# linxihui/NNLM

Measured on AMD Instinct MI355X. Metric: nnmf iterations/sec + final MSE, dense A 20000x10000 k=50, 1/2/4/8 GPU, higher is better.
Workload: dtype f32 (A fp32; cross-product operands 22-bit split-fp16 pairs; Gram / sweeps fp64); 1 GPU; nnmf(A, k=50) MSE+SCD on 20000x10000 dense A (BASELINE.json configs[1]); n=20000, m=10000, k=50, method=1, inner_max_iter=50, trace=2, protocol=default, rel_tol=-1, parallelism=1 GPU

## Files before the change

include/nnlm_mi355x.h:

```cpp
#ifndef NNLM_MI355X_H
#define NNLM_MI355X_H

#include <stddef.h>

#ifdef __cplusplus
extern "C" {
#endif

#define NNLM_ABI_VERSION 1

#define NNLM_OK 0
#define NNLM_ERR_ARG 1
#define NNLM_ERR_HIP 2
#define NNLM_ERR_INTERRUPT 3
#define NNLM_ERR_COMM 4
#define NNLM_ERR_UNSUPPORTED 5

#define NNLM_PREC_F32 0
#define NNLM_PREC_F64 1

typedef struct nnlm_callbacks {
    void *ctx;
    int (*check_interrupt)(void *ctx);
    void (*progress)(void *ctx, unsigned done, unsigned total);
// ... 169 lines not shown
int nnlm_c_nnmf_holdout_batch(const double *A, int n, int m, const long long *colptr, const int *rowidx, unsigned B, const unsigned *k,
                              const double *W_init, const double *H_init, const double alpha[3], const double beta[3], unsigned max_iter,
                              double rel_tol, int n_threads, int verbose, int show_warning, unsigned inner_max_iter, double inner_rel_tol,
                              int method, unsigned trace, double *W_out, double *H_out, double *mse_error, double *mkl_error,
                              double *target_error, double *average_epoch, int *n_trace, unsigned *n_iteration, int *warned,
                              double *holdout_mse, double *holdout_mkl, const nnlm_callbacks *cb);

int nnlm_svd(nnlm_handle *h, unsigned l, unsigned power_iters, const double *omega);
int nnlm_debug_set_svd_rotate(int form);
int nnlm_get_svd(nnlm_handle *h, unsigned k, double *sigma, double *U, double *Vt);
int nnlm_set_factors_nndsvd(nnlm_handle *h, unsigned k, int variant);
int nnlm_set_factors_nndsvd_batch(nnlm_handle *h, unsigned B, const unsigned *k, int variant);

int nnlm_profile_enable(nnlm_handle *h, int on);
int nnlm_profile_get(nnlm_handle *h, const char *name, double *total_ms, long long *launches);
int nnlm_profile_reset(nnlm_handle *h);

#define NNLM_COMM_ID_BYTES 128
#define NNLM_FORM_COLS 0
#define NNLM_FORM_REDUCE 1
int nnlm_comm_unique_id(char id[NNLM_COMM_ID_BYTES]);
int nnlm_comm_init(nnlm_handle *h, const char id[NNLM_COMM_ID_BYTES], int rank, int nranks);
int nnlm_comm_set_form(nnlm_handle *h, int form);
int nnlm_comm_info(nnlm_handle *h, int *rank, int *nranks);
int nnlm_shard_range(int n, int m, int precision, int which, int rank, int nranks, int *begin, int *end);
int nnlm_shard_cols(int ncols, int rank, int nranks, int *cpr, int *col0, int *col1);
int nnlm_debug_partial(nnlm_handle *h, int which, double *G_out, double *C_out);

int nnlm_debug_phase(nnlm_handle *h, int which, int phase, const double reg[3], unsigned inner_max_iter,
                     double inner_rel_tol, int method);
int nnlm_debug_exchange(nnlm_handle **handles, int nranks, int which, int stage);
int nnlm_debug_set_cus(int cus);
int nnlm_debug_set_xprod_waves(int waves);
int nnlm_debug_set_a_stream(int nt_from_stage);
int nnlm_xprod_plan(int ldc, int stages, int k, int cus, int force_waves, int out[8]);
int nnlm_kl_plan(int p, int k, int precision, int mask_words, int out[8]);
int nnlm_debug_alloc_limit(size_t bytes);
int nnlm_debug_poison_workspaces(int on);
int nnlm_get_info(nnlm_handle *h, const char *key, double *value);

#ifdef __cplusplus
}
#endif
#endif
```

nnlm_amd/_lib.py:

```python
from __future__ import annotations

import ctypes as C
import os

import numpy as np

_HERE = os.path.dirname(os.path.abspath(__file__))
LIB_PATH = os.path.join(_HERE, "libnnlm_mi355x.so")

NNLM_OK = 0
ERR_ARG = 1
ERR_UNSUPPORTED = 5
BATCH_MAX = 64
PREC_F32 = 0
PREC_F64 = 1
COMM_ID_BYTES = 128
FORM_COLS = 0
FORM_REDUCE = 1
FORMS = {"cols": FORM_COLS, "reduce": FORM_REDUCE}

EXPORTS = [
    "nnlm_trace_capacity", "nnlm_c_nnmf", "nnlm_c_nnlm", "nnlm_create", "nnlm_destroy", "nnlm_last_error",
    "nnlm_abi_version", "nnlm_set_matrix", "nnlm_matrix_info", "nnlm_set_factors", "nnlm_get_factors",
    "nnlm_half_step", "nnlm_iterate", "nnlm_run", "nnlm_take_sweeps", "nnlm_errors", "nnlm_sync", "nnlm_profile_enable",
    "nnlm_profile_get", "nnlm_profile_reset", "nnlm_comm_unique_id", "nnlm_comm_init", "nnlm_comm_info",
    "nnlm_shard_range", "nnlm_shard_cols", "nnlm_debug_partial", "nnlm_debug_phase", "nnlm_debug_exchange",
    "nnlm_comm_set_form", "nnlm_debug_set_cus", "nnlm_debug_set_xprod_waves", "nnlm_debug_set_a_stream", "nnlm_xprod_plan", "nnlm_kl_plan", "nnlm_get_info", "nnlm_debug_alloc_limit", "nnlm_debug_poison_workspaces", "nnlm_release_caches",
    "nnlm_set_matrix_csc", "nnlm_c_nnmf_csc", "nnlm_c_nnlm_csc",
    "nnlm_set_matrix_csc_missing", "nnlm_c_nnmf_csc_missing", "nnlm_c_nnlm_csc_missing",
    "nnlm_set_matrix_csc_kl", "nnlm_c_nnmf_csc_kl", "nnlm_c_nnlm_csc_kl",
    "nnlm_set_factors_batch", "nnlm_get_factors_batch", "nnlm_run_batch", "nnlm_c_nnmf_batch",
    "nnlm_set_matrix_holdout", "nnlm_holdout_errors", "nnlm_c_nnmf_holdout_batch",
    "nnlm_set_matrix_device", "nnlm_set_factors_device", "nnlm_get_factors_device",
    "nnlm_predict_entries", "nnlm_top_n",
    "nnlm_set_matrix_csc_batch", "nnlm_c_nnmf_csc_batch",
    "nnlm_set_matrix_csc_kl_batch", "nnlm_c_nnmf_csc_kl_batch",
    "nnlm_set_matrix_csc_missing_batch", "nnlm_c_nnmf_csc_missing_batch",
    "nnlm_set_matrix_sparse_device", "nnlm_debug_sparse_resident",
    "nnlm_set_matrix_csc_weighted", "nnlm_c_nnmf_csc_weighted", "nnlm_c_nnlm_csc_weighted",
    "nnlm_set_matrix_sparse_device_weighted", "nnlm_debug_sparse_resident_weighted",
    "nnlm_svd", "nnlm_get_svd", "nnlm_set_factors_nndsvd", "nnlm_set_factors_nndsvd_batch", "nnlm_debug_set_svd_rotate",
]
NNDSVD_VARIANTS = {"nndsvd": 0, "nndsvda": 1}
TOPN_MAX = 128
BY = {"column": 0, "row": 1}


class NnlmError(RuntimeError):
    def __init__(self, code, msg):
        super().__init__(f"libnnlm_mi355x error {code}: {msg}")
        self.code = code


class DevMatrix(C.Structure):
    _fields_ = [("ptr", C.c_void_p), ("dtype", C.c_int), ("row_stride", C.c_longlong), ("col_stride", C.c_longlong)]


class DevSparse(C.Structure):
    _fields_ = [("ptr", C.c_void_p), ("idx", C.c_void_p), ("val", C.c_void_p), ("ptr_dtype", C.c_int), ("idx_dtype", C.c_int),
                ("val_dtype", C.c_int), ("layout", C.c_int), ("nnz", C.c_longlong)]
# ... 88 lines not shown
    lib.nnlm_errors.argtypes = [vp, dp, dp, dp]
    lib.nnlm_sync.restype = C.c_int
    lib.nnlm_sync.argtypes = [vp]
    lib.nnlm_profile_enable.restype = C.c_int
    lib.nnlm_profile_enable.argtypes = [vp, C.c_int]
    lib.nnlm_profile_reset.restype = C.c_int
    lib.nnlm_profile_reset.argtypes = [vp]
    lib.nnlm_profile_get.restype = C.c_int
    lib.nnlm_profile_get.argtypes = [vp, C.c_char_p, dp, C.POINTER(C.c_longlong)]
    lib.nnlm_comm_unique_id.restype = C.c_int
    lib.nnlm_comm_unique_id.argtypes = [C.c_char_p]
    lib.nnlm_comm_init.restype = C.c_int
    lib.nnlm_comm_init.argtypes = [vp, C.c_char_p, C.c_int, C.c_int]
    lib.nnlm_comm_info.restype = C.c_int
    lib.nnlm_comm_info.argtypes = [vp, ip, ip]
    lib.nnlm_shard_range.restype = C.c_int
    lib.nnlm_shard_range.argtypes = [C.c_int, C.c_int, C.c_int, C.c_int, C.c_int, C.c_int, ip, ip]
    lib.nnlm_shard_cols.restype = C.c_int
    lib.nnlm_shard_cols.argtypes = [C.c_int, C.c_int, C.c_int, ip, ip, ip]
    lib.nnlm_debug_partial.restype = C.c_int
    lib.nnlm_debug_partial.argtypes = [vp, C.c_int, dp, dp]
    lib.nnlm_debug_phase.restype = C.c_int
    lib.nnlm_debug_phase.argtypes = [vp, C.c_int, C.c_int, dp, C.c_uint, C.c_double, C.c_int]
    lib.nnlm_debug_exchange.restype = C.c_int
    lib.nnlm_debug_exchange.argtypes = [C.POINTER(vp), C.c_int, C.c_int, C.c_int]
    lib.nnlm_comm_set_form.restype = C.c_int
    lib.nnlm_comm_set_form.argtypes = [vp, C.c_int]
    lib.nnlm_debug_set_cus.restype = C.c_int
    lib.nnlm_debug_set_cus.argtypes = [C.c_int]
    lib.nnlm_debug_set_xprod_waves.restype = C.c_int
    lib.nnlm_debug_set_xprod_waves.argtypes = [C.c_int]
    lib.nnlm_debug_set_a_stream.restype = C.c_int
    lib.nnlm_debug_set_a_stream.argtypes = [C.c_int]
    lib.nnlm_xprod_plan.restype = C.c_int
    lib.nnlm_xprod_plan.argtypes = [C.c_int, C.c_int, C.c_int, C.c_int, C.c_int, ip]
    lib.nnlm_kl_plan.restype = C.c_int
    lib.nnlm_kl_plan.argtypes = [C.c_int, C.c_int, C.c_int, C.c_int, ip]
    lib.nnlm_debug_alloc_limit.restype = C.c_int
    lib.nnlm_debug_alloc_limit.argtypes = [C.c_size_t]
    lib.nnlm_debug_poison_workspaces.restype = C.c_int
    lib.nnlm_debug_poison_workspaces.argtypes = [C.c_int]
    lib.nnlm_release_caches.restype = C.c_int
    lib.nnlm_release_caches.argtypes = []
    lib.nnlm_get_info.restype = C.c_int
    lib.nnlm_get_info.argtypes = [vp, C.c_char_p, dp]
    up = C.POINTER(C.c_uint)
    lib.nnlm_set_factors_batch.restype = C.c_int
    lib.nnlm_set_factors_batch.argtypes = [vp, C.c_uint, up, dp, dp]
    lib.nnlm_get_factors_batch.restype = C.c_int
    lib.nnlm_get_factors_batch.argtypes = [vp, dp, dp]
    lib.nnlm_run_batch.restype = C.c_int
    lib.nnlm_run_batch.argtypes = lib.nnlm_run.argtypes
    lib.nnlm_c_nnmf_batch.restype = C.c_int
    lib.nnlm_c_nnmf_batch.argtypes = [dp, C.c_int, C.c_int, C.c_uint, up, dp, dp, dp, dp, C.c_uint, C.c_double, C.c_int, C.c_int, C.c_int,
                                      C.c_uint, C.c_double, C.c_int, C.c_uint, dp, dp, dp, dp, dp, dp, ip, up, ip, C.POINTER(Callbacks)]
    lib.nnlm_c_nnmf_csc_batch.restype = C.c_int
    lib.nnlm_c_nnmf_csc_batch.argtypes = [C.c_int, C.c_int, lp, ip, dp] + lib.nnlm_c_nnmf_batch.argtypes[3:]
    lib.nnlm_set_matrix_csc_batch.restype = C.c_int
    lib.nnlm_set_matrix_csc_batch.argtypes = lib.nnlm_set_matrix_csc.argtypes
    lib.nnlm_c_nnmf_csc_kl_batch.restype = C.c_int
    lib.nnlm_c_nnmf_csc_kl_batch.argtypes = lib.nnlm_c_nnmf_csc_batch.argtypes
    lib.nnlm_set_matrix_csc_kl_batch.restype = C.c_int
    lib.nnlm_set_matrix_csc_kl_batch.argtypes = lib.nnlm_set_matrix_csc.argtypes
    lib.nnlm_set_matrix_csc_missing_batch.restype = C.c_int
    lib.nnlm_set_matrix_csc_missing_batch.argtypes = lib.nnlm_set_matrix_csc.argtypes + [lp, ip]
    lib.nnlm_c_nnmf_csc_missing_batch.restype = C.c_int
# ... 893 lines not shown
        cols = self.m if which == 1 else self.n
        G = np.zeros((self.k, self.k), order="F")
        Cm = np.zeros((self.k, cols), order="F")
        self._ck(self._lib.nnlm_debug_partial(self._h, int(which), _dp(G), _dp(Cm)))
        return np.ascontiguousarray(G), np.ascontiguousarray(Cm)

    def comm_info(self):
        r, n = C.c_int(0), C.c_int(0)
        self._ck(self._lib.nnlm_comm_info(self._h, C.byref(r), C.byref(n)))
        return r.value, n.value


def shard_range(n, m, precision, which, rank, nranks):
    b, e = C.c_int(0), C.c_int(0)
    _check(load().nnlm_shard_range(int(n), int(m), int(precision), int(which), int(rank), int(nranks), C.byref(b), C.byref(e)))
    return b.value, e.value


def shard_cols(ncols, rank, nranks):
    cpr, c0, c1 = C.c_int(0), C.c_int(0), C.c_int(0)
    _check(load().nnlm_shard_cols(int(ncols), int(rank), int(nranks), C.byref(cpr), C.byref(c0), C.byref(c1)))
    return cpr.value, c0.value, c1.value


def debug_exchange(handles, which, stage):
    arr = (C.c_void_p * len(handles))(*[h._h for h in handles])
    _check(load().nnlm_debug_exchange(arr, len(handles), int(which), int(stage)))


def debug_set_cus(cus: int):
    _check(load().nnlm_debug_set_cus(int(cus)))


def debug_set_svd_rotate(form: int):
    _check(load().nnlm_debug_set_svd_rotate(int(form)))


def debug_set_xprod_waves(waves: int):
    _check(load().nnlm_debug_set_xprod_waves(int(waves)))


A_STREAM_NONE = 2**31 - 1


def debug_set_a_stream(nt_from_stage: int):
    _check(load().nnlm_debug_set_a_stream(int(nt_from_stage)))


def xprod_plan(ldc, stages, k, cus, force_waves=0):
    out = (C.c_int * 8)()
    _check(load().nnlm_xprod_plan(int(ldc), int(stages), int(k), int(cus), int(force_waves), out))
    return dict(zip(("waves", "splits", "stages_per_split", "tiles", "blocks", "pieces", "lds_bytes"), list(out)[:7]))


KL_TILE2, KL_TILE1, KL_REG64, KL_STREAM = 0, 1, 2, 3


def kl_plan(p, k, precision, mask_words=0):
    out = (C.c_int * 8)()
    _check(load().nnlm_kl_plan(int(p), int(k), int(precision), int(mask_words), out))
    return dict(zip(("kernel", "pieces_exact", "pieces", "cols", "lds_bytes", "last_waves"), list(out)[:6]))


def debug_alloc_limit(nbytes: int):
    _check(load().nnlm_debug_alloc_limit(int(nbytes)))

# ... 14 lines not shown
```

nnlm_amd/csrc/nnlm_mi355x.hip:

```cpp
#include "../../include/nnlm_mi355x.h"
#include "common.h"
#include "k_batch.h"
#include "k_errors.h"
#include "k_generic.h"
#include "k_gram.h"
#include "k_ingest.h"
#include "k_kl.h"
#include "k_missing.h"
#include "k_prep.h"
#include "k_sweep.h"
#include "k_sweep_q.h"
#include "k_xprod.h"
#include "k_xprod16.h"
#include "tu_sweepq.h"
#include "tu_svd.h"
#include "tu_topn.h"

#include <dlfcn.h>
#include <rccl/rccl.h>

#include <algorithm>
#include <atomic>
#include <chrono>
#include <climits>
// ... 119 lines not shown
    double *spg_buf = nullptr;
    size_t spg_buf_bytes = 0;
    int spg_chunks = 0;
    int spg_workers = 0;
    unsigned long long *sweeps = nullptr;
    int sw_active = 0;
    double *host_res = nullptr;

    int rank = 0, nranks = 1;
    void *comm = nullptr;
    bool sharded = false;
    double *pack_send = nullptr;
    double *pack_all = nullptr;
    size_t pack_elems = 0;
    double *sweepq_img = nullptr;
    bool x16 = false;
    uint32_t *A16 = nullptr, *A16T = nullptr, *Y16 = nullptr;
    unsigned *maxbits = nullptr;
    int sg_which = -1, sg_par = 0, sg_nslabs = 0;
    int sg_other = -1;
    int sg_prev = -1;
    bool sg_request = false;
    double *sg_slabs = nullptr;
    int mb_par = 0;
    bool pack_ready = false;
    int *scal_exp = nullptr;
    float *What = nullptr;
    double *What64 = nullptr;
    uint32_t *W16c = nullptr, *H16c = nullptr;
    bool fuse_err = false;
    int cus_device = 0;
    int xprod_waves = 0;
    int a_stream = -1;
    int a_stream_last = -1;
    int xp_err_splits = 0;
    int xp_waves[2] = {0, 0}, xp_splits[2] = {0, 0};
    int fused_nb = 0;
    bool err_hook = false, err_need_pen = true, err_launched = false;
    unsigned *err_zero_word = nullptr;
    unsigned long long *sweeps_tmp = nullptr;

    int bB = 0, row_pad = 0;
    std::vector<int> bk, boff;
    int *boff_dev = nullptr;
    double *bG = nullptr;
    unsigned long long *bsweeps = nullptr;
    double *bpart = nullptr;
    size_t bpart_elems = 0;
    double *bres = nullptr;
    double *bsp_Hrow = nullptr;
    double *bsp_part = nullptr;
    int bspg_pairs = 0;

    bool holdout = false;
    long long ho_nnz = 0;
    long long *ho_cptr = nullptr;
    int *ho_ridx = nullptr, *ho_cidx = nullptr;
    void *ho_val = nullptr;

    int topn_slices = 0;

    int svd_l = 0, svd_LP = 0, svd_kept = 0;
    double *svdU = nullptr, *svdVt = nullptr;
    std::vector<double> svd_sigma;
    double svd_mean = 0.0;
    bool svd_mean_known = false;
// ... 117 lines not shown
static Rccl g_rccl;

static int rccl_load()
{
    if (g_rccl.lib) return NNLM_OK;
    void *lib = dlopen("librccl.so.1", RTLD_NOW | RTLD_GLOBAL);
    if (!lib) lib = dlopen("librccl.so", RTLD_NOW | RTLD_GLOBAL);
    if (!lib) lib = dlopen("/opt/rocm/lib/librccl.so.1", RTLD_NOW | RTLD_GLOBAL);
    if (!lib) return fail(nullptr, NNLM_ERR_COMM, "cannot load librccl: %s", dlerror());
    g_rccl.GetUniqueId = (decltype(g_rccl.GetUniqueId))dlsym(lib, "ncclGetUniqueId");
    g_rccl.CommInitRank = (decltype(g_rccl.CommInitRank))dlsym(lib, "ncclCommInitRank");
    g_rccl.AllReduce = (decltype(g_rccl.AllReduce))dlsym(lib, "ncclAllReduce");
    g_rccl.AllGather = (decltype(g_rccl.AllGather))dlsym(lib, "ncclAllGather");
    g_rccl.CommDestroy = (decltype(g_rccl.CommDestroy))dlsym(lib, "ncclCommDestroy");
    g_rccl.GetErrorString = (decltype(g_rccl.GetErrorString))dlsym(lib, "ncclGetErrorString");
    if (!g_rccl.GetUniqueId || !g_rccl.CommInitRank || !g_rccl.AllReduce || !g_rccl.AllGather || !g_rccl.CommDestroy)
        return fail(nullptr, NNLM_ERR_COMM, "librccl lacks a required symbol");
    g_rccl.lib = lib;
    return NNLM_OK;
}

extern "C" int nnlm_abi_version(void) { return NNLM_ABI_VERSION; }

extern "C" const char *nnlm_last_error(const nnlm_handle *h) { return h ? h->err.c_str() : g_last_error.c_str(); }

extern "C" unsigned nnlm_trace_capacity(unsigned max_iter, unsigned trace)
{
    if (trace < 1) trace = 1;
    return (unsigned)std::ceil((double)max_iter / (double)trace) + 1;
}

static std::atomic<int> g_debug_cus{0};
static std::atomic<int> g_debug_a_stream{-1};
static std::atomic<int> g_debug_xprod_waves{0};
static std::mutex g_bounce_mu;
static double *g_bounce[2] = {nullptr, nullptr};
static size_t g_bounce_bytes = 0;
static bool g_bounce_busy = false, g_bounce_atexit = false;
static void bounce_release_at_exit()
{
    for (int b = 0; b < 2; b++)
        if (g_bounce[b]) (void)hipHostFree(g_bounce[b]);
    g_bounce[0] = g_bounce[1] = nullptr;
    g_bounce_bytes = 0;
}
static bool bounce_acquire(size_t bytes, double *out[2], bool *cached)
{
    {
        std::lock_guard<std::mutex> lk(g_bounce_mu);
        if (!g_bounce_busy) {
            if (g_bounce_bytes < bytes) {
                for (int b = 0; b < 2; b++)
                    if (g_bounce[b]) (void)hipHostFree(g_bounce[b]);
                g_bounce[0] = g_bounce[1] = nullptr;
                g_bounce_bytes = 0;
                if (hipHostMalloc(&g_bounce[0], bytes) != hipSuccess || hipHostMalloc(&g_bounce[1], bytes) != hipSuccess) {
                    (void)hipGetLastError();
                    for (int b = 0; b < 2; b++)
                        if (g_bounce[b]) (void)hipHostFree(g_bounce[b]);
                    g_bounce[0] = g_bounce[1] = nullptr;
                    return false;
                }
                g_bounce_bytes = bytes;
                if (!g_bounce_atexit) {
                    g_bounce_atexit = true;
                    atexit(bounce_release_at_exit);
// ... 46 lines not shown
{
    g_debug_alloc_limit = bytes;
    return NNLM_OK;
}

static std::atomic<int> g_debug_poison{0};

extern "C" int nnlm_debug_poison_workspaces(int on)
{
    g_debug_poison = on ? 1 : 0;
    return NNLM_OK;
}

static hipError_t poison_new_gram(void *p, size_t bytes, hipStream_t st)
{
    if (!g_debug_poison.load(std::memory_order_relaxed)) return hipSuccess;
    return hipMemsetAsync(p, 0xFF, bytes, st);
}

extern "C" int nnlm_debug_set_xprod_waves(int waves)
{
    if (waves != 0 && waves != 8 && waves != 10) return fail(nullptr, NNLM_ERR_ARG, "nnlm_debug_set_xprod_waves: %d (0, 8 or 10)", waves);
    g_debug_xprod_waves = waves;
    return NNLM_OK;
}

extern "C" int nnlm_debug_set_a_stream(int nt_from_stage)
{
    if (nt_from_stage < -1) return fail(nullptr, NNLM_ERR_ARG, "nnlm_debug_set_a_stream: %d (-1, or a stage >= 0)", nt_from_stage);
    g_debug_a_stream = nt_from_stage;
    return NNLM_OK;
}

extern "C" int nnlm_debug_set_cus(int cus)
{
    if (cus < 0) return fail(nullptr, NNLM_ERR_ARG, "nnlm_debug_set_cus: %d", cus);
    g_debug_cus = cus;
    return NNLM_OK;
}

struct HandleRes {
    bool valid = false;
    int device = -1, cus = 0;
    hipStream_t stream = nullptr, stream_e = nullptr;
    hipEvent_t ev_hdone = nullptr, ev_err = nullptr, ev_xdone = nullptr;
    double *scal = nullptr, *host_res = nullptr, *sweepq_img = nullptr;
    unsigned long long *sweeps = nullptr, *sweeps_tmp = nullptr;
    unsigned *maxbits = nullptr;
    int *scal_exp = nullptr;
};
static std::mutex g_res_mu;
static HandleRes g_res;
static bool g_res_atexit = false;
static void handle_res_destroy(HandleRes &r)
{
    (void)hipFree(r.scal), (void)hipFree(r.sweeps), (void)hipHostFree(r.host_res), (void)hipFree(r.sweeps_tmp), (void)hipFree(r.sweepq_img);
    (void)hipFree(r.maxbits), (void)hipFree(r.scal_exp);
    if (r.ev_hdone) (void)hipEventDestroy(r.ev_hdone);
    if (r.ev_err) (void)hipEventDestroy(r.ev_err);
    if (r.ev_xdone) (void)hipEventDestroy(r.ev_xdone);
    if (r.stream_e) (void)hipStreamDestroy(r.stream_e);
    if (r.stream) (void)hipStreamDestroy(r.stream);
    r = HandleRes{};
}
static void handle_res_release_at_exit()
{
    if (g_res.valid) handle_res_destroy(g_res);
}

extern "C" int nnlm_create(nnlm_handle **out, int device, int precision)
{
    if (!out) return fail(nullptr, NNLM_ERR_ARG, "nnlm_create: out is NULL");
    *out = nullptr;
    if (precision != NNLM_PREC_F32 && precision != NNLM_PREC_F64) return fail(nullptr, NNLM_ERR_ARG, "nnlm_create: unknown precision %d", precision);
    int ndev = 0;
    hipError_t e = hipGetDeviceCount(&ndev);
    if (e != hipSuccess || ndev <= 0)
        return fail(nullptr, NNLM_ERR_HIP, "nnlm_create: no HIP device available (%s); libnnlm_mi355x has no CPU path", e != hipSuccess ? hipGetErrorString(e) : "device count 0");
    if (device < 0 || device >= ndev) return fail(nullptr, NNLM_ERR_ARG, "nnlm_create: device %d out of range (0..%d)", device, ndev - 1);
    HIPCHK(nullptr, hipSetDevice(device));
    HandleRes res;
    {
        std::lock_guard<std::mutex> lk(g_res_mu);
        if (g_res.valid && g_res.device == device) {
            res = g_res;
            g_res = HandleRes{};
        }
    }
    if (res.valid) {
        nnlm_handle *h = new nnlm_handle();
        h->device = device;
        h->prec = precision;
        h->cus = h->cus_device = res.cus;
        if (const int dc = g_debug_cus.load(std::memory_order_relaxed); dc > 0) h->cus = dc;
        h->xprod_waves = g_debug_xprod_waves.load(std::memory_order_relaxed);
        h->a_stream = g_debug_a_stream.load(std::memory_order_relaxed);
        h->stream = res.stream, h->stream_e = res.stream_e;
        h->ev_hdone = res.ev_hdone, h->ev_err = res.ev_err, h->ev_xdone = res.ev_xdone;
        h->scal = res.scal, h->sweeps = res.sweeps, h->host_res = res.host_res, h->sweeps_tmp = res.sweeps_tmp, h->sweepq_img = res.sweepq_img;
        h->maxbits = res.maxbits, h->scal_exp = res.scal_exp;
        const bool alive = hipMemsetAsync(h->sweeps, 0, 2 * sizeof(unsigned long long), h->stream) == hipSuccess &&
                           hipMemsetAsync(h->scal_exp, 0, 4 * sizeof(int), h->stream) == hipSuccess &&
                           hipMemsetAsync(h->maxbits, 0, 16 * sizeof(unsigned), h->stream) == hipSuccess &&
                           hipStreamSynchronize(h->stream) == hipSuccess && hipStreamSynchronize(h->stream_e) == hipSuccess;
        if (alive) {
            h->x16 = x16_enabled(precision);
            *out = h;
            return NNLM_OK;
        }
        (void)hipGetLastError();
        delete h;
        handle_res_destroy(res);
    }
    hipDeviceProp_t prop;
    HIPCHK(nullptr, hipGetDeviceProperties(&prop, device));
    if (strncmp(prop.gcnArchName, "gfx950", 6) != 0)
        return fail(nullptr, NNLM_ERR_HIP, "nnlm_create: device %d is %s; this library is built for gfx950 (MI355X) only", device, prop.gcnArchName);
    nnlm_handle *h = new nnlm_handle();
    h->device = device;
    h->prec = precision;
    h->cus = prop.multiProcessorCount > 0 ? prop.multiProcessorCount : 256;
    h->cus_device = h->cus;
    if (const int dc = g_debug_cus.load(std::memory_order_relaxed); dc > 0) h->cus = dc;
    h->xprod_waves = g_debug_xprod_waves.load(std::memory_order_relaxed);
    h->a_stream = g_debug_a_stream.load(std::memory_order_relaxed);
    if (hipStreamCreateWithFlags(&h->stream, hipStreamNonBlocking) != hipSuccess ||
        hipStreamCreateWithFlags(&h->stream_e, hipStreamNonBlocking) != hipSuccess ||
        hipEventCreateWithFlags(&h->ev_hdone, hipEventDisableTiming) != hipSuccess ||
        hipEventCreateWithFlags(&h->ev_err, hipEventDisableTiming) != hipSuccess ||
        hipEventCreateWithFlags(&h->ev_xdone, hipEventDisableTiming) != hipSuccess) {
        delete h;
        return fail(nullptr, NNLM_ERR_HIP, "nnlm_create: stream/event creation failed");
    }
    if (hipMalloc(&h->scal, 16 * sizeof(double)) != hipSuccess || hipMalloc(&h->sweeps, 2 * sizeof(unsigned long long)) != hipSuccess ||
        hipHostMalloc(&h->host_res, 16 * sizeof(double)) != hipSuccess ||
        hipMalloc(&h->sweeps_tmp, sizeof(unsigned long long)) != hipSuccess ||
        hipMalloc(&h->sweepq_img, sweepq_img_doubles(16, true) * sizeof(double)) != hipSuccess ||
        hipMalloc(&h->maxbits, 16 * sizeof(unsigned)) != hipSuccess || hipMalloc(&h->scal_exp, 4 * sizeof(int)) != hipSuccess) {
        delete h;
        return fail(nullptr, NNLM_ERR_HIP, "nnlm_create: hipMalloc failed");
    }
    if (hipMemsetAsync(h->sweeps, 0, 2 * sizeof(unsigned long long), h->stream) != hipSuccess ||
        hipMemsetAsync(h->scal_exp, 0, 4 * sizeof(int), h->stream) != hipSuccess ||
        hipMemsetAsync(h->maxbits, 0, 16 * sizeof(unsigned), h->stream) != hipSuccess || hipStreamSynchronize(h->stream) != hipSuccess) {
        const hipError_t em = hipGetLastError();
        HandleRes dead;
        dead.stream = h->stream, dead.stream_e = h->stream_e, dead.ev_hdone = h->ev_hdone, dead.ev_err = h->ev_err, dead.ev_xdone = h->ev_xdone;
        dead.scal = h->scal, dead.sweeps = h->sweeps, dead.host_res = h->host_res, dead.sweeps_tmp = h->sweeps_tmp, dead.sweepq_img = h->sweepq_img;
        dead.maxbits = h->maxbits, dead.scal_exp = h->scal_exp;
        delete h;
        handle_res_destroy(dead);
        return fail(nullptr, NNLM_ERR_HIP, "nnlm_create: clearing the handle's counters failed: %s", hipGetErrorString(em));
    }
    h->x16 = x16_enabled(precision);
    *out = h;
    return NNLM_OK;
}

// ... 2041 lines not shown
}

template <int STEP, int L>
static void launch_sweep_l(int idx, int method, const SweepArgs &a, hipStream_t s)
{
    switch (idx) {
    case 1: launch_sweep_m<1 * STEP, L>(method, a, s); break;
    case 2: launch_sweep_m<2 * STEP, L>(method, a, s); break;
    case 3: launch_sweep_m<3 * STEP, L>(method, a, s); break;
    case 4: launch_sweep_m<4 * STEP, L>(method, a, s); break;
    case 5: launch_sweep_m<5 * STEP, L>(method, a, s); break;
    case 6: launch_sweep_m<6 * STEP, L>(method, a, s); break;
    case 7: launch_sweep_m<7 * STEP, L>(method, a, s); break;
    default: launch_sweep_m<8 * STEP, L>(method, a, s); break;
    }
}

static int sweep_lanes_per_column(int ncols)
{
    const long slots = 1024L * 4;
    if (((long)ncols * 4 + 63) / 64 <= slots) return 4;
    if (((long)ncols * 2 + 63) / 64 <= slots) return 2;
    return 1;
}

static bool sweep_fast(const nnlm_handle *h) { return h->prec == NNLM_PREC_F32 && h->k <= NNLM_KQ_MAX; }

static size_t sg_slab_count(const nnlm_handle *h)
{
    const int big = h->n > h->m ? h->n : h->m;
    const int wide = (big + SWEEPQ_COLS - 1) / SWEEPQ_COLS, row = (big + 15) / 16 < h->cus ? (big + 15) / 16 : h->cus;
    return (size_t)(wide > row ? wide : row) + 1;
}
static void launch_sweep_f(nnlm_handle *h, const SweepArgs &a)
{
    const int ncols = a.ncols - a.col0, NB = (a.k + 3) / 4;
    h->sweep_wgs = 0;
    h->pack_ready = false;
    if (ncols <= 0) return;
    if (a.k <= SWEEPR_KMAX && ncols <= 32 * h->cus) {
        const int NWr = (ncols <= 16 * h->cus) ? 4 : 8;
        const int nbr = (ncols + 4 * NWr - 1) / (4 * NWr);
        h->sweep_wgs = nbr;
        h->sweep_form[h->cur_which] = 3;
        h->sweep_groups[h->cur_which] = NWr;
        nnlm_tu_sweep_r(a, nbr, NWr, h->stream);
        return;
    }
    const int ngroups = (ncols + 15) / 16, simds = 4 * h->cus;
    const int NW = ngroups > simds ? 8 : 4;
    const int nb = (ncols + 16 * NW - 1) / (16 * NW);
    h->sweep_wgs = nb;
    h->sweep_form[h->cur_which] = 2;
    h->sweep_groups[h->cur_which] = NW;
    const hipError_t ea = nnlm_tu_sweep_f(a, nb, NB, NW, h->stream);
    if (ea != hipSuccess && g_attr_err == hipSuccess) {
        g_attr_err = ea;
        g_attr_what = "sweep_scd_f_kernel";
    }
}

static void launch_sweep_q(nnlm_handle *h, const SweepArgs &a)
{
    if (h->prec == NNLM_PREC_F32) return launch_sweep_f(h, a);
    int nb = (a.ncols - a.col0 + SWEEPQ_COLS - 1) / SWEEPQ_COLS;
    const int NB = (a.k + 3) / 4;
    h->sweep_wgs = 0;
    if (nb <= 0) return;
    if (!h->pack_ready)
        sweepq_pack_kernel<<<8, 256, 0, h->stream>>>(a.Graw, a.KPg, a.k, a.r0, a.r1, NB, h->sweepq_img, 1);
    h->pack_ready = false;
    const int ngroups = (a.ncols - a.col0 + 15) / 16, simds = 4 * h->cus;
    int G = 0;
    if (ngroups > simds && a.max_iter >= 4) {
        long best = ((long)ngroups + simds - 1) / simds * 4;
        for (int g = 5; g <= SWEEPQ_WRAP_MAXG; g++) {
            if (sweepqw_lds_bytes(h->KP, NB, true, g) > (size_t)160 * 1024) break;
            const long wgs = ((long)ngroups + g - 1) / g, rounds = (wgs + h->cus - 1) / h->cus;
            if (rounds * g < best) best = rounds * g, G = g;
        }
    }
    if (G) nb = (ngroups + G - 1) / G;
    h->sweep_wgs = nb;
    h->sweep_form[h->cur_which] = G ? 1 : 0;
    h->sweep_groups[h->cur_which] = G ? G : 4;
    const hipError_t ea = G ? nnlm_tu_sweep_qw(a, h->sweepq_img, nb, NB, true, G, h->stream) : nnlm_tu_sweep_q(a, h->sweepq_img, nb, NB, true, h->stream);
    if (ea != hipSuccess && g_attr_err == hipSuccess) {
        g_attr_err = ea;
        g_attr_what = G ? "sweep_scd_qw_kernel" : "sweep_scd_q_kernel";
    }
}
// ... 2843 lines not shown
```

nnlm_amd/csrc/tu_sweepq.h:

```cpp
#pragma once
#include "k_sweep.h"

hipError_t nnlm_tu_sweep_q(const SweepArgs &a, const double *img, int nb, int NB, bool strict, hipStream_t st);
hipError_t nnlm_tu_sweep_qw(const SweepArgs &a, const double *img, int nb, int NB, bool strict, int G, hipStream_t st);
hipError_t nnlm_tu_sweep_f(const SweepArgs &a, int nb, int NB, int NW, hipStream_t st);
void nnlm_tu_colsolve_row(const SweepArgs &a, size_t g_stride, hipStream_t st);
#define SWEEPR_KMAX 50
void nnlm_tu_sweep_r(const SweepArgs &a, int nb, int NW, hipStream_t st);

struct SpmmArgs {
    const long long *ptr;
    const int *idx;
    const void *val;
    const void *Y;
    long long nnz, chunk;
    int ncols, KP, q0;
    int nworkers;
    double *C;
    int ldc;
    double *carry;
};
void nnlm_tu_spmm(const SpmmArgs &a, bool f64, hipStream_t st);
void nnlm_tu_sp_errors(const long long *ptr, const int *idx, const void *val, bool f64, int ncols, long long nnz, long long chunk, int nworkers,
                       const double *Wrow, int KP, int k, const double *H, int ldh, double *partial, int nblocks, bool miss, hipStream_t st);
int nnlm_sp_workers(long long nnz, int KP, int cus);
int nnlm_sp_lanes(int KP);
void nnlm_tu_sp_rowsums(const double *X, int ld, int ncols, int KP, double *partial, int nblocks, hipStream_t st);
void nnlm_tu_sp_err_final(const double *s, const double *GW, const double *GH, const double *wsum, const double *hsum, int k, int KP, double *out,
                          hipStream_t st);
void nnlm_tu_sp_batch_errors(const long long *ptr, const int *idx, const void *val, bool f64, int ncols, long long nnz, long long chunk, int nwaves,
                             const double *Wrow, const double *Hrow, int KP, const int *off, int B, unsigned long long amask, double *partial,
                             hipStream_t st);
#define SPB_BATCH_MAX 64
int nnlm_spb_waves(long long nnz, int cus);
long long nnlm_spb_chunk(long long nnz, int nwaves);
void nnlm_tu_sp_batch_final(const double *s, const double *GW, const double *GH, const double *wsum, const double *hsum, const int *off, int B, int KP,
                            unsigned long long amask, double *out, hipStream_t st);

// ... 91 lines not shown
```

Baseline: 1774 iterations/s.

## Add wide 32-column-per-wave SCD sweep kernel using 32x32 bf16 MFMA

After: 1786 iterations/s, median of 6. About the same (+0.7%).

```diff
diff --git a/include/nnlm_mi355x.h b/include/nnlm_mi355x.h
--- a/include/nnlm_mi355x.h
+++ b/include/nnlm_mi355x.h
@@ -225,6 +225,8 @@
 int nnlm_debug_exchange(nnlm_handle **handles, int nranks, int which, int stage);
 int nnlm_debug_set_cus(int cus);
 int nnlm_debug_set_xprod_waves(int waves);
+int nnlm_debug_set_sweep_wide(int wide);
+int nnlm_sweep_plan(int k, int ncols, int cus, int wide, int masked, int *out);
 int nnlm_debug_set_a_stream(int nt_from_stage);
 int nnlm_xprod_plan(int ldc, int stages, int k, int cus, int force_waves, int out[8]);
 int nnlm_kl_plan(int p, int k, int precision, int mask_words, int out[8]);
diff --git a/nnlm_amd/_lib.py b/nnlm_amd/_lib.py
--- a/nnlm_amd/_lib.py
+++ b/nnlm_amd/_lib.py
@@ -25,7 +25,7 @@
     "nnlm_half_step", "nnlm_iterate", "nnlm_run", "nnlm_take_sweeps", "nnlm_errors", "nnlm_sync", "nnlm_profile_enable",
     "nnlm_profile_get", "nnlm_profile_reset", "nnlm_comm_unique_id", "nnlm_comm_init", "nnlm_comm_info",
     "nnlm_shard_range", "nnlm_shard_cols", "nnlm_debug_partial", "nnlm_debug_phase", "nnlm_debug_exchange",
-    "nnlm_comm_set_form", "nnlm_debug_set_cus", "nnlm_debug_set_xprod_waves", "nnlm_debug_set_a_stream", "nnlm_xprod_plan", "nnlm_kl_plan", "nnlm_get_info", "nnlm_debug_alloc_limit", "nnlm_debug_poison_workspaces", "nnlm_release_caches",
+    "nnlm_comm_set_form", "nnlm_debug_set_cus", "nnlm_debug_set_xprod_waves", "nnlm_debug_set_a_stream", "nnlm_debug_set_sweep_wide", "nnlm_sweep_plan", "nnlm_xprod_plan", "nnlm_kl_plan", "nnlm_get_info", "nnlm_debug_alloc_limit", "nnlm_debug_poison_workspaces", "nnlm_release_caches",
     "nnlm_set_matrix_csc", "nnlm_c_nnmf_csc", "nnlm_c_nnlm_csc",
     "nnlm_set_matrix_csc_missing", "nnlm_c_nnmf_csc_missing", "nnlm_c_nnlm_csc_missing",
     "nnlm_set_matrix_csc_kl", "nnlm_c_nnmf_csc_kl", "nnlm_c_nnlm_csc_kl",
@@ -180,6 +180,10 @@
     lib.nnlm_debug_set_xprod_waves.argtypes = [C.c_int]
     lib.nnlm_debug_set_a_stream.restype = C.c_int
     lib.nnlm_debug_set_a_stream.argtypes = [C.c_int]
+    lib.nnlm_debug_set_sweep_wide.restype = C.c_int
+    lib.nnlm_debug_set_sweep_wide.argtypes = [C.c_int]
+    lib.nnlm_sweep_plan.restype = C.c_int
+    lib.nnlm_sweep_plan.argtypes = [C.c_int, C.c_int, C.c_int, C.c_int, C.c_int, ip]
     lib.nnlm_xprod_plan.restype = C.c_int
     lib.nnlm_xprod_plan.argtypes = [C.c_int, C.c_int, C.c_int, C.c_int, C.c_int, ip]
     lib.nnlm_kl_plan.restype = C.c_int
@@ -1139,6 +1143,16 @@
     _check(load().nnlm_debug_set_cus(int(cus)))
 
 
+def debug_set_sweep_wide(wide: int):
+    _check(load().nnlm_debug_set_sweep_wide(int(wide)))
+
+
+def sweep_plan(k: int, ncols: int, cus: int, wide: int = -1, masked: bool = False):
+    out = (C.c_int * 3)()
+    _check(load().nnlm_sweep_plan(int(k), int(ncols), int(cus), int(wide), int(bool(masked)), out))
+    return int(out[0]), int(out[1]), int(out[2])
+
+
 def debug_set_svd_rotate(form: int):
     _check(load().nnlm_debug_set_svd_rotate(int(form)))
 
diff --git a/nnlm_amd/csrc/k_sweep_w.h b/nnlm_amd/csrc/k_sweep_w.h
--- /dev/null
+++ b/nnlm_amd/csrc/k_sweep_w.h
@@ -0,0 +1,292 @@
+#pragma once
+#include "k_sweep_f.h"
+
+typedef float f32x16 __attribute__((ext_vector_type(16)));
+
+__host__ __device__ static inline size_t sweepw_lds_bytes(int KP, int KP2)
+{
+    const size_t g = ((size_t)KP2 * (KP2 + 1) + KP2) * 8, xi = (size_t)128 * (KP + 2) * 8;
+    return ((g > xi ? g : xi) + 15) / 16 * 16;
+}
+
+__device__ __forceinline__ f32x16 sw_mfma3(u32x4 a, u32x4 b, f32x16 c)
+{
+    return __builtin_amdgcn_mfma_f32_32x32x16_bf16(__builtin_bit_cast(bf16x8, a), __builtin_bit_cast(bf16x8, b), c, 0, 0, 0);
+}
+
+template <int hv> __device__ __forceinline__ float sw_share(float ea, float eb)
+{
+    if constexpr (hv == 0) return __uint_as_float(__builtin_amdgcn_permlane32_swap(__float_as_uint(ea), __float_as_uint(eb), false, false)[0]);
+    else return __uint_as_float(__builtin_amdgcn_permlane32_swap(__float_as_uint(eb), __float_as_uint(ea), false, false)[1]);
+}
+
+template <int NA2, int NB, bool HAS_MASK>
+__device__ __forceinline__ void sweepw32_body(const SweepArgs &a, unsigned char *smem)
+{
+    constexpr int NT = (NB + 3) / 4, KP = 16 * NT, KP2 = 32 * NA2, GP = KP2 + 1, XS = KP + 2, COLS = 128, THREADS = 256;
+    static_assert(NB <= 8 * NA2 && NB > 8 * (NA2 - 1) && NB >= 1, "NA2 = ceil(NB / 8)");
+    double *xl = (double *)smem;
+    double *gl = (double *)smem;
+    double *rinv = gl + KP2 * GP;
+    const int tid = threadIdx.x, lane = tid & 63, wave = tid >> 6;
+    const int h = lane >> 5, j = lane & 31;
+    const int g4 = lane >> 4, c16 = lane & 15;
+    const int k = a.k;
+    const int col_base = a.col0 + blockIdx.x * COLS;
+    const int cl = 32 * wave + j, col = col_base + cl;
+    const bool in_range = col < a.ncols;
+    const int cc = in_range ? col : a.col0;
+
+#ifdef SWEEPF_TIMING
+    const long long tm0 = __builtin_readcyclecounter();
+#endif
+    unsigned long long mword = 0ull;
+    if (HAS_MASK) mword = a.mask[cc];
+    f32x16 nu[NA2], x[NA2];
+#pragma unroll
+    for (int T = 0; T < NA2; T++)
+#pragma unroll
+        for (int r = 0; r < 16; r++) {
+            const int q = 32 * T + 8 * (r / 4) + 4 * h + r % 4;
+            x[T][r] = (q < k && in_range) ? (float)a.X[(size_t)q * a.ldx + col] : 0.0f;
+        }
+    auto coord64 = [&](int T, int s2, int g, int r) { return 32 * T + 8 * (2 * s2 + (g & 1)) + 4 * (g >> 1) + r; };
+    f64x4 a64[NA2][2][2];
+    int col64[2], cc64[2];
+    bool in64[2];
+#pragma unroll
+    for (int ch = 0; ch < 2; ch++) {
+        col64[ch] = col_base + 32 * wave + 16 * ch + c16;
+        in64[ch] = col64[ch] < a.ncols;
+        cc64[ch] = in64[ch] ? col64[ch] : a.col0;
+    }
+#pragma unroll
+    for (int T = 0; T < NA2; T++)
+#pragma unroll
+        for (int s2 = 0; s2 < 2; s2++)
+#pragma unroll
+            for (int ch = 0; ch < 2; ch++) a64[T][s2][ch] = f64x4{0, 0, 0, 0};
+    for (int s = 0; s < a.nslabs; s++) {
+#pragma unroll
+        for (int ch = 0; ch < 2; ch++) {
+            const double *cs = a.Cx + (size_t)s * a.slab_stride + cc64[ch];
+#pragma unroll
+            for (int T = 0; T < NA2; T++)
+#pragma unroll
+                for (int s2 = 0; s2 < 2; s2++)
+#pragma unroll
+                    for (int r = 0; r < 4; r++) {
+                        const int q = coord64(T, s2, g4, r);
+                        a64[T][s2][ch][r] += (q < k) ? cs[(size_t)q * a.ldc] : 0.0;
+                    }
+        }
+    }
+    constexpr bool XB_EARLY = !HAS_MASK;
+    auto load_xb = [&](int c, int ch) { return (4 * c + g4 < k && in64[ch]) ? a.X[(size_t)(4 * c + g4) * a.ldx + col64[ch]] : 0.0; };
+    double xb[XB_EARLY ? NB : 1][2];
+    if constexpr (XB_EARLY) {
+#pragma unroll
+        for (int c = 0; c < NB; c++)
+#pragma unroll
+            for (int ch = 0; ch < 2; ch++) xb[c][ch] = load_xb(c, ch);
+    }
+    sweepf_build_gprime<KP2, THREADS>(a, gl, rinv);
+#ifdef SWEEPF_TIMING
+    const long long tmA = __builtin_readcyclecounter();
+#endif
+    const unsigned long long kmask = (k >= 64) ? ~0ull : ((1ull << k) - 1ull);
+    bool act = in_range && !(HAS_MASK && ((mword & kmask) == kmask));
+
+    u32x4 Ares[NA2][NB][2];
+#pragma unroll
+    for (int T = 0; T < NA2; T++)
+#pragma unroll
+        for (int b = 0; b < NB; b++)
+#pragma unroll
+            for (int m = 0; m < 2; m++) {
+                Ares[T][b][m] = sf_split_a(-(float)gl[(32 * T + j) * GP + 4 * b + 2 * m + (h ^ (b & 1))]);
+                asm("" : "+a"(Ares[T][b][m]));
+            }
+#ifdef SWEEPF_TIMING
+    const long long tmB = __builtin_readcyclecounter();
+#endif
+    {
+#pragma unroll
+        for (int T = 0; T < NA2; T++)
+#pragma unroll
+            for (int s2 = 0; s2 < 2; s2++)
+#pragma unroll
+                for (int ch = 0; ch < 2; ch++)
+#pragma unroll
+                    for (int r = 0; r < 4; r++) {
+                        const int q = coord64(T, s2, g4, r);
+                        const double v = a64[T][s2][ch][r];
+                        a64[T][s2][ch][r] = (q < k) ? ((a.r2 != 0) ? a.r2 - v : -v) * rinv[q] : 0.0;
+                    }
+#pragma unroll
+        for (int c = 0; c < NB; c++) {
+            const int q = 4 * c + g4;
+            const double xb0 = XB_EARLY ? xb[XB_EARLY ? c : 0][0] : load_xb(c, 0), xb1 = XB_EARLY ? xb[XB_EARLY ? c : 0][1] : load_xb(c, 1);
+#pragma unroll
+            for (int T = 0; T < NA2; T++)
+#pragma unroll
+                for (int s2 = 0; s2 < 2; s2++) {
+                    const double av = gl[coord64(T, s2, c16 & 3, c16 >> 2) * GP + q];
+                    a64[T][s2][0] = __builtin_amdgcn_mfma_f64_16x16x4f64(av, xb0, a64[T][s2][0], 0, 0, 0);
+                    a64[T][s2][1] = __builtin_amdgcn_mfma_f64_16x16x4f64(av, xb1, a64[T][s2][1], 0, 0, 0);
+                }
+        }
+#pragma unroll
+        for (int T = 0; T < NA2; T++)
+#pragma unroll
+            for (int s2 = 0; s2 < 2; s2++)
+#pragma unroll
+                for (int r = 0; r < 4; r++) {
+                    const auto p = __builtin_amdgcn_permlane16_swap(__float_as_uint((float)a64[T][s2][0][r]), __float_as_uint((float)a64[T][s2][1][r]), false, false);
+                    nu[T][8 * s2 + r] = __uint_as_float(p[0]);
+                    nu[T][8 * s2 + 4 + r] = __uint_as_float(p[1]);
+                }
+        if (HAS_MASK) {
+#pragma unroll
+            for (int T = 0; T < NA2; T++)
+#pragma unroll
+                for (int r = 0; r < 16; r++) {
+                    const int q = 32 * T + 8 * (r / 4) + 4 * h + r % 4;
+                    if (q < 64 && ((mword >> q) & 1ull)) x[T][r] = 0.0f, nu[T][r] = 1e30f;
+                }
+        }
+    }
+#ifdef SWEEPF_TIMING
+    const long long tmC = __builtin_readcyclecounter();
+#endif
+    float Ls[NA2][4][2], nsel[2];
+    f32x2 Lp[NA2][4][2];
+    float neg_huge = -3.0e38f;
+    asm volatile("" : "+v"(neg_huge));
+#pragma unroll
+    for (int T = 0; T < NA2; T++)
+#pragma unroll
+        for (int s = 0; s < 4; s++) {
+            const int q0 = 32 * T + 8 * s + 4 * h;
+            const double *gb = gl + q0 * GP + q0;
+            Ls[T][s][0] = -(float)gb[1 * GP + 0], Ls[T][s][1] = -(float)gb[3 * GP + 2];
+            Lp[T][s][0] = f32x2{-(float)gb[2 * GP + 0], -(float)gb[3 * GP + 0]};
+            Lp[T][s][1] = f32x2{-(float)gb[2 * GP + 1], -(float)gb[3 * GP + 1]};
+        }
+    nsel[0] = (h == 0) ? -1.0f : 0.0f, nsel[1] = (h == 1) ? -1.0f : 0.0f;
+    __syncthreads();
+
+    auto write_col = [&]() {
+#pragma unroll
+        for (int T = 0; T < NA2; T++)
+#pragma unroll
+            for (int r = 0; r < 16; r++) {
+                const int q = 32 * T + 8 * (r / 4) + 4 * h + r % 4;
+                if (q >= KP) continue;
+                xl[cl * XS + q] = in_range ? (double)x[T][r] : 0.0;
+            }
+    };
+    if (!act) write_col();
+
+    const float tol = (float)a.rel_tol, tolh = 0.5f * tol, tolhe = 0.5f * tol * (float)NNLM_TINY;
+    unsigned t = 0;
+    int t_lane = 0;
+    bool go = a.max_iter > 0 && __any(act);
+    unsigned long long flagmask = 0ull;
+    u32x4 pb[2] = {u32x4{0u, 0u, 0u, 0u}, u32x4{0u, 0u, 0u, 0u}};
+    auto step = [&](auto bc, auto tc) {
+        constexpr int B = decltype(bc)::value, T = B / 8, s = (B % 8) / 2, hv = B % 2, R = 4 * s, TN = ((B + 1) % NB) / 8, PB = (B + NB - 1) % NB;
+        constexpr bool TEST = decltype(tc)::value;
+        const float xo0 = x[T][R], xo1 = x[T][R + 1], xo2 = x[T][R + 2], xo3 = x[T][R + 3];
+        const float e0 = __builtin_amdgcn_fmed3f(xo0, nu[T][R], neg_huge);
+        __builtin_amdgcn_sched_barrier(0);
+#pragma unroll
+        for (int o = 1; o < NA2; o++) nu[(T + o) % NA2] = sw_mfma3(Ares[(T + o) % NA2][PB][0], pb[0], nu[(T + o) % NA2]);
+        __builtin_amdgcn_sched_barrier(0);
+        const float n1 = __builtin_fmaf(Ls[T][s][0], e0, nu[T][R + 1]);
+        f32x2 n23 = __builtin_elementwise_fma(Lp[T][s][0], f32x2{e0, e0}, f32x2{nu[T][R + 2], nu[T][R + 3]});
+        const float e1 = __builtin_fminf(xo1, n1);
+        n23 = __builtin_elementwise_fma(Lp[T][s][1], f32x2{e1, e1}, n23);
+        __builtin_amdgcn_sched_barrier(0);
+        const f32x2 x01 = __builtin_elementwise_fma(f32x2{e0, e1}, f32x2{nsel[hv], nsel[hv]}, f32x2{xo0, xo1});
+        __builtin_amdgcn_sched_barrier(0);
+        const float e2 = __builtin_fminf(xo2, n23[0]);
+        const float n3 = __builtin_fmaf(Ls[T][s][1], e2, n23[1]);
+        const float e3 = __builtin_fminf(xo3, n3);
+        const f32x2 x23 = __builtin_elementwise_fma(f32x2{e2, e3}, f32x2{nsel[hv], nsel[hv]}, f32x2{xo2, xo3});
+        if (TEST) {
+            const float ev[4] = {e0, e1, e2, e3}, xv[4] = {xo0, xo1, xo2, xo3};
+            unsigned long long mv = 0ull;
+#pragma unroll
+            for (int r = 0; r < 4; r++) mv |= __ballot(__builtin_fabsf(ev[r]) > __builtin_fmaf(tolh, __builtin_fmaf(2.0f, xv[r], -ev[r]), tolhe));
+            flagmask |= mv & (0xFFFFFFFFull << (32 * hv));
+        }
+        x[T][R] = x01[0], x[T][R + 1] = x01[1], x[T][R + 2] = x23[0], x[T][R + 3] = x23[1];
+        __builtin_amdgcn_sched_barrier(0);
+#pragma unroll
+        for (int o = 1; o < NA2; o++) nu[(T + o) % NA2] = sw_mfma3(Ares[(T + o) % NA2][PB][1], pb[1], nu[(T + o) % NA2]);
+        __builtin_amdgcn_sched_barrier(0);
+        pb[0] = sf_split_b(sw_share<hv>(e0, e1));
+        nu[TN] = sw_mfma3(Ares[TN][B][0], pb[0], nu[TN]);
+        __builtin_amdgcn_sched_barrier(0);
+        pb[1] = sf_split_b(sw_share<hv>(e2, e3));
+        nu[TN] = sw_mfma3(Ares[TN][B][1], pb[1], nu[TN]);
+        __builtin_amdgcn_sched_barrier(0);
+    };
+    auto moved = [&]() -> unsigned { return (unsigned)((flagmask | (flagmask >> 32)) & 0xFFFFFFFFull); };
+#ifdef SWEEPF_TIMING
+    const long long tm1 = __builtin_readcyclecounter();
+#endif
+    while (go) {
+        flagmask = (0.0f > tol) ? ~0ull : 0ull;
+        step(std::integral_constant<int, 0>{}, std::true_type{});
+        if (__any(act && !((moved() >> j) & 1u))) {
+            sq_for<1, NB>([&](auto bc) { step(bc, std::true_type{}); });
+        } else {
+            sq_for<1, NB>([&](auto bc) { step(bc, std::false_type{}); });
+        }
+        if (act) {
+            t_lane++;
+            if (!((moved() >> j) & 1u)) {
+                write_col();
+                act = false;
+            }
+        }
+        t++;
+        go = t < a.max_iter && __any(act);
+    }
+#ifdef SWEEPF_TIMING
+    const long long tm2 = __builtin_readcyclecounter();
+#endif
+    if (act) write_col();
+    if (HAS_MASK && in_range) {
+        int hh = h;
+        asm volatile("" : "+v"(hh));
+        for (int T = 0; T < NA2; T++)
+            for (int r = 0; r < 16; r++) {
+                const int q = 32 * T + 8 * (r / 4) + 4 * hh + r % 4;
+                if (q < k && ((mword >> q) & 1ull)) xl[cl * XS + q] = a.X[(size_t)q * a.ldx + col];
+            }
+    }
+    __syncthreads();
+
+    sweepq_epilogue<NT, COLS, 4>(a, xl, COLS, col_base, (int)blockIdx.x);
+#ifdef SWEEPF_TIMING
+    if (a.op_mode == 98 && tid == 0 && blockIdx.x == 0) {
+        long long *tmo = (long long *)a.op;
+        tmo[0] = tm1 - tm0, tmo[1] = tm2 - tm1, tmo[2] = __builtin_readcyclecounter() - tm2, tmo[3] = t;
+        tmo[4] = tmA - tm0, tmo[5] = tmB - tmA, tmo[6] = tmC - tmB, tmo[7] = tm1 - tmC;
+    }
+#endif
+    {
+        const long long tot = wave_sum_ll((h == 0) ? (long long)t_lane : 0ll);
+        if (lane == 0 && tot) atomicAdd(a.sweeps, (unsigned long long)tot);
+    }
+}
+
+template <int NA2, int NB, bool HAS_MASK>
+__global__ __launch_bounds__(256, 1) void sweep_scd_w_kernel(const SweepArgs a)
+{
+    extern __shared__ __attribute__((aligned(16))) unsigned char sw_smem[];
+    sweepw32_body<NA2, NB, HAS_MASK>(a, sw_smem);
+}
diff --git a/nnlm_amd/csrc/nnlm_mi355x.hip b/nnlm_amd/csrc/nnlm_mi355x.hip
--- a/nnlm_amd/csrc/nnlm_mi355x.hip
+++ b/nnlm_amd/csrc/nnlm_mi355x.hip
@@ -175,6 +175,7 @@
     int cus_device = 0;
     int xprod_waves = 0;
     int a_stream = -1;
+    int sweep_wide = -1;
     int a_stream_last = -1;
     int xp_err_splits = 0;
     int xp_waves[2] = {0, 0}, xp_splits[2] = {0, 0};
@@ -358,6 +359,7 @@
 
 static std::atomic<int> g_debug_cus{0};
 static std::atomic<int> g_debug_a_stream{-1};
+static std::atomic<int> g_debug_sweep_wide{-1};
 static std::atomic<int> g_debug_xprod_waves{0};
 static std::mutex g_bounce_mu;
 static double *g_bounce[2] = {nullptr, nullptr};
@@ -470,6 +472,13 @@
     return NNLM_OK;
 }
 
+extern "C" int nnlm_debug_set_sweep_wide(int wide)
+{
+    if (wide < -1 || wide > 1) return fail(nullptr, NNLM_ERR_ARG, "nnlm_debug_set_sweep_wide: %d (-1, 0 or 1)", wide);
+    g_debug_sweep_wide = wide;
+    return NNLM_OK;
+}
+
 extern "C" int nnlm_debug_set_cus(int cus)
 {
     if (cus < 0) return fail(nullptr, NNLM_ERR_ARG, "nnlm_debug_set_cus: %d", cus);
@@ -533,6 +542,7 @@
         if (const int dc = g_debug_cus.load(std::memory_order_relaxed); dc > 0) h->cus = dc;
         h->xprod_waves = g_debug_xprod_waves.load(std::memory_order_relaxed);
         h->a_stream = g_debug_a_stream.load(std::memory_order_relaxed);
+        h->sweep_wide = g_debug_sweep_wide.load(std::memory_order_relaxed);
         h->stream = res.stream, h->stream_e = res.stream_e;
         h->ev_hdone = res.ev_hdone, h->ev_err = res.ev_err, h->ev_xdone = res.ev_xdone;
         h->scal = res.scal, h->sweeps = res.sweeps, h->host_res = res.host_res, h->sweeps_tmp = res.sweeps_tmp, h->sweepq_img = res.sweepq_img;
@@ -562,6 +572,7 @@
     if (const int dc = g_debug_cus.load(std::memory_order_relaxed); dc > 0) h->cus = dc;
     h->xprod_waves = g_debug_xprod_waves.load(std::memory_order_relaxed);
     h->a_stream = g_debug_a_stream.load(std::memory_order_relaxed);
+    h->sweep_wide = g_debug_sweep_wide.load(std::memory_order_relaxed);
     if (hipStreamCreateWithFlags(&h->stream, hipStreamNonBlocking) != hipSuccess ||
         hipStreamCreateWithFlags(&h->stream_e, hipStreamNonBlocking) != hipSuccess ||
         hipEventCreateWithFlags(&h->ev_hdone, hipEventDisableTiming) != hipSuccess ||
@@ -2669,31 +2680,42 @@
     const int wide = (big + SWEEPQ_COLS - 1) / SWEEPQ_COLS, row = (big + 15) / 16 < h->cus ? (big + 15) / 16 : h->cus;
     return (size_t)(wide > row ? wide : row) + 1;
 }
+extern "C" int nnlm_sweep_plan(int k, int ncols, int cus, int wide, int masked, int *out)
+{
+    if (k < 1 || k > NNLM_KQ_MAX || ncols < 1 || cus < 1 || wide < -1 || wide > 1 || !out)
+        return fail(nullptr, NNLM_ERR_ARG, "nnlm_sweep_plan: k %d, %d columns, %d compute units, wide %d", k, ncols, cus, wide);
+    const int ngroups = (ncols + 15) / 16, simds = 4 * cus;
+    const bool fits = !(masked && k > SWEEPW_KMAX_MASKED);
+    if (fits && (wide == 1 || (wide == -1 && ngroups > simds && ngroups <= 2 * simds && ncols >= 4096))) {
+        out[0] = 4, out[1] = 4, out[2] = (ncols + 127) / 128;
+    } else if (k <= SWEEPR_KMAX && ncols <= 32 * cus) {
+        out[1] = (ncols <= 16 * cus) ? 4 : 8;
+        out[0] = 3, out[2] = (ncols + 4 * out[1] - 1) / (4 * out[1]);
+    } else {
+        out[1] = ngroups > simds ? 8 : 4;
+        out[0] = 2, out[2] = (ncols + 16 * out[1] - 1) / (16 * out[1]);
+    }
+    return NNLM_OK;
+}
 static void launch_sweep_f(nnlm_handle *h, const SweepArgs &a)
 {
     const int ncols = a.ncols - a.col0, NB = (a.k + 3) / 4;
     h->sweep_wgs = 0;
     h->pack_ready = false;
     if (ncols <= 0) return;
-    if (a.k <= SWEEPR_KMAX && ncols <= 32 * h->cus) {
-        const int NWr = (ncols <= 16 * h->cus) ? 4 : 8;
-        const int nbr = (ncols + 4 * NWr - 1) / (4 * NWr);
-        h->sweep_wgs = nbr;
-        h->sweep_form[h->cur_which] = 3;
-        h->sweep_groups[h->cur_which] = NWr;
-        nnlm_tu_sweep_r(a, nbr, NWr, h->stream);
+    int plan[3];
+    if (nnlm_sweep_plan(a.k, ncols, h->cus, h->sweep_wide, a.mask != nullptr, plan) != NNLM_OK) return;
+    h->sweep_form[h->cur_which] = plan[0];
+    h->sweep_groups[h->cur_which] = plan[1];
+    h->sweep_wgs = plan[2];
+    if (plan[0] == 3) {
+        nnlm_tu_sweep_r(a, plan[2], plan[1], h->stream);
         return;
     }
-    const int ngroups = (ncols + 15) / 16, simds = 4 * h->cus;
-    const int NW = ngroups > simds ? 8 : 4;
-    const int nb = (ncols + 16 * NW - 1) / (16 * NW);
-    h->sweep_wgs = nb;
-    h->sweep_form[h->cur_which] = 2;
-    h->sweep_groups[h->cur_which] = NW;
-    const hipError_t ea = nnlm_tu_sweep_f(a, nb, NB, NW, h->stream);
+    const hipError_t ea = plan[0] == 4 ? nnlm_tu_sweep_w(a, plan[2], NB, h->stream) : nnlm_tu_sweep_f(a, plan[2], NB, plan[1], h->stream);
     if (ea != hipSuccess && g_attr_err == hipSuccess) {
         g_attr_err = ea;
-        g_attr_what = "sweep_scd_f_kernel";
+        g_attr_what = plan[0] == 4 ? "sweep_scd_w_kernel" : "sweep_scd_f_kernel";
     }
 }
 
diff --git a/nnlm_amd/csrc/tu_sweepq.h b/nnlm_amd/csrc/tu_sweepq.h
--- a/nnlm_amd/csrc/tu_sweepq.h
+++ b/nnlm_amd/csrc/tu_sweepq.h
@@ -4,6 +4,8 @@
 hipError_t nnlm_tu_sweep_q(const SweepArgs &a, const double *img, int nb, int NB, bool strict, hipStream_t st);
 hipError_t nnlm_tu_sweep_qw(const SweepArgs &a, const double *img, int nb, int NB, bool strict, int G, hipStream_t st);
 hipError_t nnlm_tu_sweep_f(const SweepArgs &a, int nb, int NB, int NW, hipStream_t st);
+#define SWEEPW_KMAX_MASKED 56
+hipError_t nnlm_tu_sweep_w(const SweepArgs &a, int nb, int NB, hipStream_t st);
 void nnlm_tu_colsolve_row(const SweepArgs &a, size_t g_stride, hipStream_t st);
 #define SWEEPR_KMAX 50
 void nnlm_tu_sweep_r(const SweepArgs &a, int nb, int NW, hipStream_t st);
diff --git a/nnlm_amd/csrc/tu_sweepw.hip b/nnlm_amd/csrc/tu_sweepw.hip
--- /dev/null
+++ b/nnlm_amd/csrc/tu_sweepw.hip
@@ -0,0 +1,35 @@
+#include "tu_sweepq.h"
+#include "k_sweep_w.h"
+
+template <int NA2, int NB, bool M> static hipError_t launch_k(const SweepArgs &a, int nb, hipStream_t st)
+{
+    const int lds = (int)sweepw_lds_bytes(16 * ((NB + 3) / 4), 32 * NA2);
+    const hipError_t e = hipFuncSetAttribute((const void *)sweep_scd_w_kernel<NA2, NB, M>, hipFuncAttributeMaxDynamicSharedMemorySize, lds);
+    sweep_scd_w_kernel<NA2, NB, M><<<nb, 256, lds, st>>>(a);
+    return e;
+}
+template <int NA2, int NB> static hipError_t launch_m(const SweepArgs &a, int nb, hipStream_t st)
+{
+    return a.mask ? launch_k<NA2, NB, true>(a, nb, st) : launch_k<NA2, NB, false>(a, nb, st);
+}
+hipError_t nnlm_tu_sweep_w(const SweepArgs &a, int nb, int NB, hipStream_t st)
+{
+    switch (NB) {
+    case 1: return launch_m<1, 1>(a, nb, st);
+    case 2: return launch_m<1, 2>(a, nb, st);
+    case 3: return launch_m<1, 3>(a, nb, st);
+    case 4: return launch_m<1, 4>(a, nb, st);
+    case 5: return launch_m<1, 5>(a, nb, st);
+    case 6: return launch_m<1, 6>(a, nb, st);
+    case 7: return launch_m<1, 7>(a, nb, st);
+    case 8: return launch_m<1, 8>(a, nb, st);
+    case 9: return launch_m<2, 9>(a, nb, st);
+    case 10: return launch_m<2, 10>(a, nb, st);
+    case 11: return launch_m<2, 11>(a, nb, st);
+    case 12: return launch_m<2, 12>(a, nb, st);
+    case 13: return launch_m<2, 13>(a, nb, st);
+    case 14: return launch_m<2, 14>(a, nb, st);
+    case 15: return a.mask ? hipErrorInvalidValue : launch_k<2, 15, false>(a, nb, st);
+    default: return a.mask ? hipErrorInvalidValue : launch_k<2, 16, false>(a, nb, st);
+    }
+}
```
